# JCSaltFish/PBRPathTracer

Hardware: AMD Instinct MI355X
Metric: Msamples/s (pixels*spp/s) (higher is better)
Workload: dtype f32; 1 GPU; Cornell box (12 tris, no textures), 1280x720, 8 bounces, 256 spp; width=1280, height=720, max_depth=8, triangles=12, bvh_nodes=1, bvh_depth=1, parallelism=single GPU, exchange=none

## Files before the change

### include/ptk.h

```cpp
#ifndef PTK_H
#define PTK_H

#include <stddef.h>
#include <stdint.h>

#ifdef __cplusplus
extern "C" {
#endif

#define PTK_OK 0
#define PTK_ERR_BAD_ARG (-1)
#define PTK_ERR_HIP (-2)
#define PTK_ERR_RCCL (-3)
#define PTK_ERR_LIMIT (-4)

#define PTK_TILE 16
#ifndef PTK_MAX_BVH_DEPTH
#define PTK_MAX_BVH_DEPTH 32
#endif

typedef struct ptk_material {
    int32_t type;
    float diffuse[3];
    float specular[3];
// ... 418 lines not shown
int ptk_probe_unpack(ptk_ctx* ctx, int world, const float* host_packed , float* host_image);

int ptk_set_option(ptk_ctx* ctx, const char* name, double value);

int ptk_last_render_ms(ptk_ctx* ctx, float* ms, int* launches);
int ptk_last_kernel_ms(ptk_ctx* ctx, float* trace_ms, float* accumulate_ms);
int ptk_kernel_log(ptk_ctx* ctx, int capacity);
#define PTK_TRACE_NONE 0
#define PTK_TRACE_BVH 1
#define PTK_TRACE_FLAT 2
#define PTK_TRACE_FLAT_PLAIN 3
int ptk_trace_variant(ptk_ctx* ctx, int* variant);
int ptk_scene_is_plain(const ptk_scene_desc* scene);
int ptk_scene_is_lambert(const ptk_scene_desc* scene);
int ptk_trace_is_lambert(ptk_ctx* ctx, int* lambert);
int ptk_flat_zero_class(const float edges[6]);
int ptk_flat_zero_mask(int zero_class);
int ptk_flat_classes(ptk_ctx* ctx, int32_t out[16]);
int ptk_flat_rect_pair(const float rec_a[9], const float rec_b[9]);
int ptk_flat_rect_pairs(ptk_ctx* ctx, int32_t out[8], int32_t* num_pairs );
int ptk_kernel_log_read(ptk_ctx* ctx, float* trace_ms, int max_entries, int* num_entries);
int ptk_collect_stats(ptk_ctx* ctx, uint32_t first_sample, uint32_t spp_count, uint64_t seed, ptk_stats* out);
int ptk_bvh_info(ptk_ctx* ctx, int32_t* num_nodes, int32_t* depth , int32_t* num_leaf_tris);
int ptk_upload_timing(ptk_ctx* ctx, double* ms4, int* built_on_device );
int ptk_bvh_layout(ptk_ctx* ctx, int32_t* node_width, int32_t* node_bytes, int32_t* stack_need);

int ptk_download_bvh(ptk_ctx* ctx, float* nodes16, int32_t* leaf_order);

int ptk_probe_hits(ptk_ctx* ctx, int n, const float* ro, const float* rd, int32_t* tri, float* tuv);
int ptk_probe_primary_dirs(ptk_ctx* ctx, float* host_out );
// ... 8 lines not shown
```

### pbrpathtracer_amd/csrc/ptk_api.hip

```cpp
#include <hip/hip_runtime.h>
#include <hip/hip_gl_interop.h>
#include <dlfcn.h>

#include <algorithm>
#include <chrono>
#include <cmath>
#include <cstring>

#include "bvh_build.h"
#include "bvh_device.h"
#include "ptk_ctx.h"
#include "ptk_stage.h"
#include "ptk_device_fn.h"
#include "ptk_adaptive.h"
#include "ptk_refit.h"
#include "ptk_flat_mt.h"

using namespace ptk;

namespace {

inline float as_float(int32_t i) { float f; std::memcpy(&f, &i, 4); return f; }

void normalize3(const float* in, float* out)
// ... 180 lines not shown
struct AdaptiveRound
{
    AdaptiveParams a;
    ConvergeParams cp;
    bool init;
};

int run_passes(ptk_ctx* c, uint32_t first, uint32_t spp, uint64_t seed, bool stats, float* accum, uint8_t* rgb8,
               const uint32_t* exit_flag, bool timed, const AdaptiveRound* ad = nullptr)
{
    RenderParams p;
    fill_params(c, p, first, spp, seed);
    p.accum = accum; p.rgb8 = rgb8; p.exit_flag = exit_flag;
    if (const int rc = use_primary_cache(c, p); rc != PTK_OK) return rc;
    p.plain = (c->opt_plain_kernel && c->scene_plain && p.flat_count > 0 && p.primary_hit != nullptr) ? 1 : 0;
    if (p.plain && c->opt_flat_rect_pairs) p.plain = 2;
    p.lambert = (p.plain && c->opt_lambert_kernel && c->scene_lambert) ? 1 : 0;
    if (!c->pixel_rng_valid || c->pixel_rng_seed != seed)
    {
        launch_pixel_rng((uint32_t)seed, (uint32_t)(seed >> 32), c->width * c->height, c->d_pixel_rng, c->stream);
        HIPCHK(c, hipGetLastError());
        c->pixel_rng_seed = seed; c->pixel_rng_valid = true;
        c->inputs_dirty = true;
    }
    p.pixel_rng = c->d_pixel_rng;
    GlMapping glmap{ c };
    uint8_t* handoff = nullptr;
    if (rgb8 == c->d_rgb8)
    {
        handoff = c->out_host_dev ? c->out_host_dev : c->out_device;
        if (!handoff && c->gl_res)
// ... 133 lines not shown
        p.resolve_samples = (float)(first + done + n);
        const long long items = (long long)tiles * 4 * num_chunks;
        if (items > (1ll << 30)) return fail(c, PTK_ERR_LIMIT, "too many work items in one pass");
        p.num_items = (int)items;
        const int pi = c->last_passes < ptk_ctx::kMaxTimedPasses ? c->last_passes : -1;
        if (timed && pi >= 0) HIPCHK(c, hipEventRecord(c->ev[pi][0], tstream));
        const int kl = (!stats && (size_t)(2 * c->klog_n + 1) < c->klog_ev.size()) ? c->klog_n : -1;
        if (kl >= 0) HIPCHK(c, hipEventRecord(c->klog_ev[2 * kl], tstream));
        p.queues = overlap ? c->d_queues2[b] : c->d_queues;
        if (c->opt_contract == 1 && !stats) fma::launch_trace(p, tiles * 4, c->resident_waves, tstream, false);
        else if (c->opt_contract == 2 && !stats) fast::launch_trace(p, tiles * 4, c->resident_waves, tstream, false);
        else launch_trace(p, tiles * 4, c->resident_waves, tstream, stats);
        HIPCHK(c, hipGetLastError());
        c->last_trace_variant = p.flat_count <= 0 ? PTK_TRACE_BVH : ((p.plain && !stats) ? PTK_TRACE_FLAT_PLAIN : PTK_TRACE_FLAT);
        c->last_trace_lambert = p.flat_count > 0 && p.plain && p.lambert && !stats;
        if (timed && pi >= 0) HIPCHK(c, hipEventRecord(c->ev[pi][1], tstream));
        if (kl >= 0) { HIPCHK(c, hipEventRecord(c->klog_ev[2 * kl + 1], tstream)); c->klog_n = kl + 1; }
        if (overlap)
        {
            HIPCHK(c, hipEventRecord(c->ev_trace_done[b], tstream));
            HIPCHK(c, hipStreamWaitEvent(c->stream, c->ev_trace_done[b], 0));
        }
        if (ad) launch_accumulate_adaptive(p, ad->a, tiles, c->stream);
        else launch_accumulate(p, tiles, c->stream);
        HIPCHK(c, hipGetLastError());
        if (timed && pi >= 0) HIPCHK(c, hipEventRecord(c->ev[pi][2], c->stream));
        if (overlap)
        {
            HIPCHK(c, hipEventRecord(c->ev_acc_done[b], c->stream));
            c->acc_pending[b] = true;
// ... 543 lines not shown

int ptk_trace_variant(ptk_ctx* c, int* variant)
{
    if (!c || !variant) return PTK_ERR_BAD_ARG;
    *variant = c->last_trace_variant;
    return PTK_OK;
}

int ptk_trace_is_lambert(ptk_ctx* c, int* lambert)
{
    if (!c || !lambert) return PTK_ERR_BAD_ARG;
    *lambert = c->last_trace_lambert ? 1 : 0;
    return PTK_OK;
}

int ptk_set_camera(ptk_ctx* c, const float pos[3], const float dir[3], const float up[3],
                   float focal, float fovy_deg, float focal_dist, float aperture)
{
    if (!c || !pos || !dir || !up) return PTK_ERR_BAD_ARG;
    for (int a = 0; a < 3; a++)
        if (!(std::fabs(pos[a]) < 2.305843e18f)) return fail(c, PTK_ERR_LIMIT, "camera position is not finite or exceeds 2^61");
    for (int a = 0; a < 3; a++) c->cam_pos[a] = pos[a];
    normalize3(dir, c->cam_dir);
    normalize3(up, c->cam_up);
    c->focal = focal;
    if (c->focal <= 0.0f) c->focal = 0.1f;
    c->fovy = fovy_deg;
    if (c->fovy <= 0.0f) c->fovy = 0.1f;
    else if (c->fovy >= 180.0f) c->fovy = 179.5;
    c->focal_dist = focal_dist;
// ... 715 lines not shown
        return PTK_OK;
    }
    if (!std::strcmp(name, "flat_rect_pairs"))
    {
        const int use = value != 0.0 ? 1 : 0;
        if (use != c->opt_flat_rect_pairs && c->have_scene && c->d_flat_tris)
        {
            HIPCHK(c, hipSetDevice(c->device));
            launch_flat_classes(c->d_flat_tris, c->num_tris, c->opt_flat_zero_classes, use, c->stream);
            HIPCHK(c, hipGetLastError());
            c->inputs_dirty = true;
        }
        c->opt_flat_rect_pairs = use;
        return PTK_OK;
    }
    if (!std::strcmp(name, "device_build"))
    {
        c->opt_device_build = value != 0.0;
        return PTK_OK;
    }
    if (!std::strcmp(name, "primary_cache"))
    {
        c->opt_primary_cache = value != 0.0;
        return PTK_OK;
    }
    if (!std::strcmp(name, "pass_bytes"))
    {
        if (!(value >= 1 << 20 && value <= 32.0 * 1073741824.0)) return fail(c, PTK_ERR_BAD_ARG, "pass_bytes must be in [1 MiB, 32 GiB]");
        c->opt_pass_bytes = (size_t)value;
        return PTK_OK;
// ... 48 lines not shown
```

### pbrpathtracer_amd/csrc/ptk_ctx.h

```cpp
#pragma once
#include <hip/hip_runtime.h>

#include <atomic>
#include <mutex>
#include <string>
#include <vector>

#include "ptk_features.h"

typedef struct ncclComm* ncclComm_t;
namespace ptk { struct RaysBlock; }

struct ptk_ctx {
    int device = 0;
    hipStream_t stream = nullptr;
    bool own_stream = false;
    std::string error;
    std::mutex err_mu;

    float4* d_flat_tris = nullptr;
    float4 *d_nodes = nullptr, *d_tris = nullptr, *d_shade = nullptr, *d_mats = nullptr, *d_lights = nullptr;
    int4* d_texinfo = nullptr;
    uint32_t* d_texels = nullptr;
    int num_nodes = 0, num_tris = 0, num_lights = 0, bvh_depth = 0, bvh_stack = 0, num_leaf_tris = 0;
// ... 16 lines not shown
    float4* d_refit_side = nullptr;
    float* d_geo_stage = nullptr; size_t geo_stage_floats = 0;
    uint32_t* d_geo_red = nullptr;
    uint32_t* h_geo_red = nullptr;
    hipStream_t geo_stream = nullptr;
    hipEvent_t ev_geo_t[5] = { nullptr, nullptr, nullptr, nullptr, nullptr };
    bool geo_done_recorded = false, lights_stale = false;
    uint32_t geo_updates = 0;
    double sah_built = 0.0, sah_now = 0.0; bool sah_now_pending = false;
    float bvh_pad = 0.0f;
    bool scene_plain = false;
    int opt_plain_kernel = 1;
    bool scene_lambert = false;
    int opt_lambert_kernel = 1;
    int opt_flat_rect_pairs = 1;
    int opt_flat_zero_classes = 1;
    int last_trace_variant = PTK_TRACE_NONE;
    bool last_trace_lambert = false;

    float cam_pos[3] = { 0, 0, 0 }, cam_dir[3] = { 0, 0, 1 }, cam_up[3] = { 0, 1, 0 };
    float focal = 0.1f, fovy = 90.0f, focal_dist = 5.0f, aperture = 0.0f;
    float cam_right[3] = { 1, 0, 0 };
    bool primary_dirty = true;

    int width = 0, height = 0, max_depth = 3;
    float4* d_primary = nullptr;
    float4* d_primary_hit = nullptr;
    float4* d_primary_rd = nullptr;
    uint2* d_pixel_rng = nullptr;
    uint64_t pixel_rng_seed = 0; bool pixel_rng_valid = false;
    bool primary_hit_dirty = true, scene_has_opacity = false;
    int opt_primary_cache = 1;
// ... 253 lines not shown
```

### pbrpathtracer_amd/csrc/ptk_kernels.hip

```cpp

#include "ptk_device_fn.h"
#include "ptk_flat_mt.h"

namespace ptk {
#if PTK_CONTRACT >= 2
namespace fast {
#elif PTK_CONTRACT
namespace fma {
#endif

#define PTK_TRACE_BLOCK 64
#ifndef PTK_TRACE_WAVES
#define PTK_TRACE_WAVES 5
#endif
#ifndef PTK_TRACE_WAVES_PLAIN
#define PTK_TRACE_WAVES_PLAIN 5
#endif
#ifndef PTK_TRACE_WAVES_BVH
#define PTK_TRACE_WAVES_BVH 4
#endif

struct RayPair { f2 ox, oy, oz, dx, dy, dz; };

template <unsigned ZM>
// ... 225 lines not shown
    W.begin(camPos0, V(0.0f, 0.0f, 1.0f), 0, stack, 0.0f);
    W.occl_tri = -1;
    Walk WS;
    WS.begin(camPos0, V(0.0f, 0.0f, 1.0f), 0, stack, 0.0f);
    WS.occl_tri = -1;
    v3 L = V(0.0f, 0.0f, 0.0f), T = V(1.0f, 1.0f, 1.0f);
    v3 Tdi = V(0.0f, 0.0f, 0.0f), nextDir = V(0.0f, 0.0f, 1.0f);
    int depth = 0, iter = 0;
    bool inside = false;
    uint32_t ray = 0;
    int st = ST_NEED;

    float4* const samples_u = uniform_ptr(P.samples);
    const int num_nodes_u = __builtin_amdgcn_readfirstlane(P.num_nodes);
    const float scene_bound_u = __int_as_float(__builtin_amdgcn_readfirstlane(__float_as_int(P.scene_bound)));
#define PTK_FINISH_PATH()                                                                         \
    do {                                                                                          \
        samples_u[out_idx] = make_float4(L.x, L.y, L.z, 0.0f);                                    \
        st = ST_NEED;                                                                             \
    } while (0)

#define PTK_WALK_DONE()                                                                           \
    do {                                                                                          \
        if (STATS) { cnt.rays++; cnt.max_nodes = max(cnt.max_nodes, cnt.cur_nodes); cnt.cur_nodes = 0; }     \
        ray++;                                                                                    \
        const bool hit_ = W.best.tri != PTK_NOHIT;                                                \
        if (W.occl_tri >= 0)                                                                      \
        {                                                                                         \
                                \
            if (STATS) cnt.shadow++;                                                              \
            if (!(hit_ && W.best.tri != W.occl_tri)) L = add(L, Tdi);                             \
            W.occl_tri = -1;                                                                      \
            W.begin(W.ro, nextDir, num_nodes_u, stack, scene_bound_u);                                   \
        }                                                                                         \
        else if (!hit_ || (FLAT && !STATS && !((LAMBERT ? depth : iter) < P.max_depth))) PTK_FINISH_PATH();       \
        else st = ST_SHADE;                                                                       \
    } while (0)

    int debt_shade = 0, debt_gen = 0;
    for (;;)
    {
        bool deal = true;
        if (FLAT)
        {
            const int n_need = __popcll(__ballot(st == ST_NEED)), nt = __popcll(__ballot(st == ST_TRAV));
            const int ns = __popcll(__ballot(st == ST_SHADE)), ng = PLAIN ? 0 : __popcll(__ballot(st == ST_GEN));
            deal = nt == 0 || nt * 8 < (ns + n_need) * P.flat_shade_w || (!PLAIN && nt * 8 < (ng + n_need) * P.flat_gen_w);
        }
        if (!FLAT || deal)
        {
            unsigned long long m_need = __ballot(st == ST_NEED);
            while (m_need)
            {
// ... 24 lines not shown
        const unsigned long long m_gen = PLAIN ? 0ull : __ballot(st == ST_GEN);
        const int n_trav = __popcll(m_trav), n_shade = __popcll(m_shade), n_gen = __popcll(m_gen);
        const int n_live = n_trav + n_shade + n_gen;
        if (n_live == 0) break;

        bool run_shade = n_trav == 0 && n_shade >= n_gen && n_shade > 0;
        bool run_gen = n_trav == 0 && !run_shade;
        if (FLAT)
        {
            const int sc_trav = n_trav * 8, sc_shade = n_shade * P.flat_shade_w, sc_gen = n_gen * P.flat_gen_w;
            if (n_trav > 0 && sc_trav >= sc_shade && sc_trav >= sc_gen)
            {
                if (STATS && lane == 0) { cnt.walk_iters++; cnt.walk_lanes += (uint32_t)n_trav; }
                if (st == ST_TRAV)
                {
                    typedef float f4v __attribute__((ext_vector_type(4)));
                    typedef const __attribute__((address_space(4))) f4v* cf4;
                    const cf4 ct = (cf4)(uintptr_t)P.flat_tris;
                    const bool shadow = WS.occl_tri >= 0;
                    const uint32_t bounce_ray = shadow ? ray + 1u : ray;
                    RayPair R;
                    R.ox = f2{ W.ro.x, WS.ro.x }; R.oy = f2{ W.ro.y, WS.ro.y }; R.oz = f2{ W.ro.z, WS.ro.z };
                    R.dx = f2{ W.rd.x, WS.rd.x }; R.dy = f2{ W.rd.y, WS.rd.y }; R.dz = f2{ W.rd.z, WS.rd.z };
                    constexpr bool ZERO_CLASSES = PLAIN && !STATS && !PTK_CONTRACT;
                    typedef const __attribute__((address_space(4))) unsigned long long* cu64;
                    const unsigned long long classes = ZERO_CLASSES ? *(cu64)(uintptr_t)(P.flat_tris + FLAT_CLASSES_AT) : 0ull;
#ifdef PTK_RECT_UNIT
                    static_assert(ZERO_CLASSES, "the pair unit holds the exact PLAIN kernels only");
                    const unsigned long long pairs = *(cu64)(uintptr_t)(P.flat_tris + FLAT_PAIRS_AT);
                    const int n_pairs = (int)(pairs >> 32) & 15;
                    for (int j = 0; j < n_pairs; j++)
                    {
                        const f4v a0 = ct[j * 2 * TRI_F4], a1 = ct[j * 2 * TRI_F4 + 1], a2 = ct[j * 2 * TRI_F4 + 2];
                        f2 aA, uA, vA, tA, aB, uB, vB, tB;
#define PTK_RECT_KIND(c) tri_math_rect<c>(W, R, a0.x, a0.y, a0.z, a1.z, a1.w, a2.x, aA, uA, vA, tA, aB, uB, vB, tB); break;
                        switch ((unsigned)(pairs >> (j * 4)) & 15u)
                        {
                            case 1: PTK_RECT_KIND(1) case 2: PTK_RECT_KIND(2) case 3: PTK_RECT_KIND(3) case 4: PTK_RECT_KIND(4) case 5: PTK_RECT_KIND(5)
                            default: PTK_RECT_KIND(6)
                        }
#undef PTK_RECT_KIND
                        tri_accept_rect(W, WS, shadow, aA, tA, uA, vA, uB, vB, __float_as_int(a2.y));
                    }
                    for (int k = n_pairs * 2; k < P.flat_count; k++)
#else
                    for (int k = 0; k < P.flat_count; k++)
#endif
                    {
                        const f4v a0 = ct[k * TRI_F4], a1 = ct[k * TRI_F4 + 1], a2 = ct[k * TRI_F4 + 2];
                        const float4 t0 = make_float4(a0.x, a0.y, a0.z, a0.w), t1 = make_float4(a1.x, a1.y, a1.z, a1.w),
                                     t2 = make_float4(a2.x, a2.y, a2.z, a2.w);
#define PTK_ZERO_CLASS(c) case c: tri_math_pair<ZERO_CLASSES ? ptk_mt::flat_zero_mask(c) : 0u>(W, R, t0, t1, t2, ma, mu, mv, mt); break;
                        if (ZERO_CLASSES)
                        {
                            f2 ma, mu, mv, mt;
                            switch ((unsigned)(classes >> (k * 4)) & 15u)
                            {
                                PTK_ZERO_CLASS(1) PTK_ZERO_CLASS(2) PTK_ZERO_CLASS(3) PTK_ZERO_CLASS(4) PTK_ZERO_CLASS(5)
                                PTK_ZERO_CLASS(6) PTK_ZERO_CLASS(7) PTK_ZERO_CLASS(8) PTK_ZERO_CLASS(9) PTK_ZERO_CLASS(10)
                                PTK_ZERO_CLASS(11) PTK_ZERO_CLASS(12) PTK_ZERO_CLASS(13) PTK_ZERO_CLASS(14) PTK_ZERO_CLASS(15)
                                default: tri_math_pair<0u>(W, R, t0, t1, t2, ma, mu, mv, mt); break;
                            }
                            (void)tri_accept_pair<STATS, PLAIN>(P, W, WS, shadow, ma, mu, mv, mt, t2, rng, bounce_ray, ray, cnt);
                        }
                        else
                            (void)tri_test_pair<STATS, PLAIN>(P, W, WS, R, shadow, t0, t1, t2, rng, bounce_ray, ray, cnt);
#undef PTK_ZERO_CLASS
                    }
                    if (shadow)
                    {
                        if (STATS) { cnt.rays++; cnt.shadow++; }
                        if (!(WS.best.tri != PTK_NOHIT && WS.best.tri != WS.occl_tri)) L = add(L, Tdi);
                        WS.occl_tri = -1;
                        ray++;
                    }
                    W.node = NODE_EXIT;
                    PTK_WALK_DONE();
                }
                continue;
            }
            run_shade = n_shade > 0 && (sc_shade >= sc_gen || n_gen == 0);
            run_gen = !run_shade;
        }
        else if (n_trav > 0)
        {
            int ds = __builtin_amdgcn_readfirstlane(debt_shade), dg = __builtin_amdgcn_readfirstlane(debt_gen);
            unsigned long long m_tq = __ballot(W.tri_left > 0), m_nr = __ballot(W.node >= 0);
            bool want_shade = false, want_gen = false;
            const WalkParams WP = walk_params(P);
            NodeRec nrec;
            request_node(WP, W, nrec);
            do
// ... 16 lines not shown
                want_shade = (ns > 0) & (ds * 8 >= WP.shade_thr * (nl - ns));
                want_gen = (ng > 0) & (dg * 8 >= WP.gen_thr * (nl - ng));
                if (want_shade | want_gen | (nt == 0)) break;
            } while (true);
            if (want_shade) run_shade = true;
            else if (want_gen) run_gen = __ballot(st == ST_NEED) == 0ull;
            debt_shade = ds; debt_gen = dg;
            if (!run_shade && !run_gen) continue;
        }
        if (run_shade) debt_shade = 0; else debt_gen = 0;
        if (run_shade)
        {
            if (STATS) { const uint32_t nsx = (uint32_t)__popcll(__ballot(st == ST_SHADE)); if (lane == 0) { cnt.shade_execs++; cnt.shade_lanes += nsx; } }
            if (st == ST_SHADE)
            {
                if (depth < 0)
                {
                    const uint2 pr = P.pixel_rng[pix];
                    const float4 c = P.primary_hit[pix], r = P.primary_rd[pix];
                    rng.inc = pr.y;
                    rng.state = hash32(P.first_sample + sample_abs + pr.x);
                    rng.key = rng.state;
                    rng.state = rng.state * (747796405u * 747796405u) + rng.inc * (747796405u + 1u);
                    L = V(0.0f, 0.0f, 0.0f); T = V(1.0f, 1.0f, 1.0f);
                    depth = 0; iter = 0; inside = false; ray = 1;
                    W.occl_tri = -1;
                    if (STATS) cnt.started++;
                    W.ro = camPos0; W.rd = V(r.x, r.y, r.z);
                    W.best.tri = __float_as_int(c.x); W.best.t = c.y; W.best.u = c.z; W.best.v = c.w;
                    W.node = NODE_EXIT; W.top = stack; W.tri_left = 0;
                }
                const bool ended = shade_interaction<STATS, FLAT, PLAIN, LAMBERT>(P, W, WS, stack, rng, L, T, Tdi, nextDir, depth, iter, inside, ray, cnt);
                if (ended) PTK_FINISH_PATH();
                else st = ST_TRAV;
            }
        }
        else if (!PLAIN)
        {
            if (STATS) { const uint32_t ngx = (uint32_t)__popcll(__ballot(st == ST_GEN)); if (lane == 0) { cnt.gen_execs++; cnt.gen_lanes += ngx; } }
            if (st == ST_GEN)
            {
                const uint2 pr = P.pixel_rng[pix];
                const uint32_t pkey = pr.x;
                rng.inc = pr.y;
                rng.state = hash32(P.first_sample + sample_abs + pkey);
                rng.key = rng.state;
                L = V(0.0f, 0.0f, 0.0f); T = V(1.0f, 1.0f, 1.0f);
                depth = 0; iter = 0; inside = false; ray = 0;
                W.occl_tri = -1;
// ... 6 lines not shown
                if (P.aperture != 0.0f)
                {
                    float angle = (float)((double)r1 * 2. * PTK_PI_D);
                    float radius = sqrt_ieee(r2);
                    float sn, cs;
                    sincos_2pi(angle, sn, cs);
                    float offx = (cs * radius) * P.aperture, offy = (sn * radius) * P.aperture;
                    ro = add(camPos0, add(muls(camRight, offx), muls(camUp, offy)));
                }
                v3 rd = normalize(sub(focalPoint, ro));
                W.begin(ro, rd, P.num_nodes, stack, P.scene_bound);
                st = ST_TRAV;
            }
        }
    }
#undef PTK_WALK_DONE
#undef PTK_FINISH_PATH
    if (STATS)
    {
        atomicAdd(&P.stats[0], (unsigned long long)cnt.started);
        atomicAdd(&P.stats[1], (unsigned long long)cnt.rays);
        atomicAdd(&P.stats[2], (unsigned long long)cnt.shadow);
        atomicAdd(&P.stats[3], (unsigned long long)cnt.nodes);
        atomicAdd(&P.stats[4], (unsigned long long)cnt.tris);
        atomicAdd(&P.stats[5], (unsigned long long)cnt.shaded);
        atomicAdd(&P.stats[6], (unsigned long long)cnt.tex);
        atomicMax(&P.stats[15], (unsigned long long)cnt.max_nodes);
        if (lane == 0)
        {
            atomicAdd(&P.stats[7], (unsigned long long)cnt.walk_iters);
            atomicAdd(&P.stats[8], (unsigned long long)cnt.walk_lanes);
            atomicAdd(&P.stats[9], (unsigned long long)cnt.shade_execs);
            atomicAdd(&P.stats[10], (unsigned long long)cnt.shade_lanes);
            atomicAdd(&P.stats[11], (unsigned long long)cnt.gen_execs);
            atomicAdd(&P.stats[12], (unsigned long long)cnt.gen_lanes);
            atomicAdd(&P.stats[13], (unsigned long long)cnt.tri_execs);
            atomicAdd(&P.stats[14], (unsigned long long)cnt.tri_lanes);
        }
    }
}

#if !PTK_CONTRACT
void launch_trace_plain(bool lambert, int blocks, hipStream_t stream, const RenderParams* dp);
void launch_trace_rect(bool lambert, int blocks, hipStream_t stream, const RenderParams* dp);
#endif
#ifdef PTK_PLAIN_UNIT
#if PTK_CONTRACT
#error "the PLAIN unit belongs to the exact build: the contracted builds keep their PLAIN kernels in ptk_kernels.hip"
#endif
#ifdef PTK_RECT_UNIT
void launch_trace_rect(bool lambert, int blocks, hipStream_t stream, const RenderParams* dp)
#else
void launch_trace_plain(bool lambert, int blocks, hipStream_t stream, const RenderParams* dp)
#endif
{
    if (lambert) hipLaunchKernelGGL((trace_kernel<false, true, true, true>), dim3(blocks), dim3(PTK_TRACE_BLOCK), 0, stream, dp);
    else hipLaunchKernelGGL((trace_kernel<false, true, true>), dim3(blocks), dim3(PTK_TRACE_BLOCK), 0, stream, dp);
}
#else

__global__ __launch_bounds__(PTK_BLOCK) void probe_math_kernel(int op, const float* __restrict__ in, float* __restrict__ out, int n)
{
    const int i = blockIdx.x * PTK_BLOCK + threadIdx.x;
    if (i >= n) return;
    const float x = in[i];
// ... 48 lines not shown
    QueueGeometry geo = {};
    geo.w[QG_NUM_CHUNKS] = p.num_chunks; geo.w[QG_WORLD] = p.world; geo.w[QG_RANK] = p.rank;
    geo.w[QG_TILES_X] = p.tiles_x; geo.w[QG_CHUNK] = p.chunk; geo.w[QG_SPP] = (int)p.spp;
    if (!(p.flat_count > 0) && PTK_TRACE_WAVES_BVH != 4) resident_waves = resident_waves / 16 * 4 * PTK_TRACE_WAVES_BVH;
    if (p.flat_count > 0 && PTK_TRACE_WAVES != 4) resident_waves = resident_waves / 16 * 4 * ((p.plain && !stats) ? PTK_TRACE_WAVES_PLAIN : PTK_TRACE_WAVES);
    if (p.persistent < 0) p.persistent = padded > 4 * resident_waves ? 1 : 0;
    const int generations = p.persistent ? std::max(1, std::min(p.generations, padded / resident_waves)) : 1;
    const int blocks = p.persistent ? resident_waves * generations : padded;
    geo.w[QG_QUOTA] = generations > 1 ? blocks : 0;
    hipLaunchKernelGGL(queue_init_kernel, dim3(1), dim3(64), 0, stream, p.queues, geo, p.live_count, p);
    const RenderParams* dp = queue_block_params(p.queues);
    const bool flat = p.flat_count > 0;
#if !PTK_CONTRACT
    if (stats && flat) hipLaunchKernelGGL((trace_kernel<true, true, false>), dim3(blocks), dim3(PTK_TRACE_BLOCK), 0, stream, dp);
    else if (stats) hipLaunchKernelGGL((trace_kernel<true, false, false>), dim3(blocks), dim3(PTK_TRACE_BLOCK), 0, stream, dp);
    else if (flat && p.plain == 2) launch_trace_rect(p.lambert != 0, blocks, stream, dp);
    else if (flat && p.plain) launch_trace_plain(p.lambert != 0, blocks, stream, dp);
    else
#else
    if (flat && p.plain && p.lambert) hipLaunchKernelGGL((trace_kernel<false, true, true, true>), dim3(blocks), dim3(PTK_TRACE_BLOCK), 0, stream, dp);
    else if (flat && p.plain) hipLaunchKernelGGL((trace_kernel<false, true, true>), dim3(blocks), dim3(PTK_TRACE_BLOCK), 0, stream, dp);
    else
#endif
    if (flat) hipLaunchKernelGGL((trace_kernel<false, true, false>), dim3(blocks), dim3(PTK_TRACE_BLOCK), 0, stream, dp);
    else hipLaunchKernelGGL((trace_kernel<false, false, false>), dim3(blocks), dim3(PTK_TRACE_BLOCK), 0, stream, dp);
}

#endif

#if PTK_CONTRACT
// ... 4 lines not shown
```

### pbrpathtracer_amd/ptk.py

```python
from __future__ import annotations

import ctypes as C
import threading
import os
from typing import Optional

import numpy as np

_HERE = os.path.dirname(os.path.abspath(__file__))
LIB_PATH = os.path.join(_HERE, "libptk.so")
if os.environ.get("PTK_DEV_TOOLS") == "1" and os.environ.get("PTK_LIB_PATH", "").startswith(os.path.join(_HERE, "libptk_")):
    LIB_PATH = os.environ["PTK_LIB_PATH"]

PTK_OK = 0
PTK_TILE = 16
PTK_MAX_BVH_DEPTH = 32

MATERIAL_DTYPE = np.dtype([
    ("type", np.int32), ("diffuse", np.float32, 3), ("specular", np.float32, 3),
    ("emissive", np.float32, 3), ("emissive_intensity", np.float32), ("roughness", np.float32),
    ("reflectiveness", np.float32), ("translucency", np.float32), ("ior", np.float32),
    ("tex", np.int32, 6)], align=False)
TEXTURE_DTYPE = np.dtype([("width", np.int32), ("height", np.int32), ("offset", np.int64)])
assert MATERIAL_DTYPE.itemsize == 84 and TEXTURE_DTYPE.itemsize == 16
# ... 104 lines not shown


_lib = None

SYMBOLS = [
    "ptk_create", "ptk_destroy", "ptk_upload_scene", "ptk_update_materials", "ptk_set_camera", "ptk_set_frame", "ptk_set_tile",
    "ptk_reset", "ptk_render", "ptk_resolve_rgb8", "ptk_read_accum", "ptk_write_accum", "ptk_samples",
    "ptk_request_exit", "ptk_synchronize", "ptk_last_error", "ptk_accum_device_ptr", "ptk_rgb8_device_ptr",
    "ptk_bind_accum", "ptk_set_stream", "ptk_gather_accum", "ptk_set_option", "ptk_last_render_ms",
    "ptk_last_kernel_ms", "ptk_collect_stats",
    "ptk_bvh_info", "ptk_bvh_layout", "ptk_upload_timing", "ptk_download_bvh", "ptk_probe_hits", "ptk_probe_primary_dirs", "ptk_probe_math", "ptk_probe_direct", "ptk_host_alloc", "ptk_host_free",
    "ptk_packed_floats", "ptk_packed_layout", "ptk_comm_unique_id", "ptk_comm_init", "ptk_comm_destroy",
    "ptk_gather_wait", "ptk_read_gathered", "ptk_gathered_device_ptr", "ptk_probe_pack", "ptk_probe_unpack",
    "ptk_bind_out_image", "ptk_bind_out_device", "ptk_bind_gl_buffer", "ptk_comm_info", "ptk_kernel_log", "ptk_kernel_log_read",
    "ptk_debug_stall_exchange", "ptk_render_adaptive", "ptk_read_sample_counts", "ptk_read_moments",
    "ptk_trace_variant", "ptk_scene_is_plain", "ptk_scene_is_lambert", "ptk_trace_is_lambert",
    "ptk_flat_zero_class", "ptk_flat_zero_mask", "ptk_flat_classes", "ptk_flat_rect_pair", "ptk_flat_rect_pairs",
    "ptk_feature_info", "ptk_render_features", "ptk_read_feature", "ptk_feature_device_ptr", "ptk_pick",
    "ptk_update_geometry", "ptk_update_geometry_device", "ptk_geometry_info", "ptk_geometry_timing",
    "ptk_trace_rays", "ptk_trace_rays_device", "ptk_last_rays_ms",
    "ptk_intersect_rays", "ptk_intersect_rays_device", "ptk_occluded_rays", "ptk_occluded_rays_device", "ptk_last_hits_ms",
    "ptk_closest_points", "ptk_closest_points_device", "ptk_last_closest_ms", "ptk_closest_stats",
    "ptk_crossings_rays", "ptk_crossings_rays_device", "ptk_contains_points", "ptk_contains_points_device",
    "ptk_inside_default_dirs", "ptk_signed_distance", "ptk_signed_distance_device", "ptk_last_crossings_ms",
    "ptk_multihit_rays", "ptk_multihit_rays_device", "ptk_last_multihit_ms",
    "ptk_denoise_planes", "ptk_denoise_planes_device", "ptk_denoise_frame", "ptk_read_denoised", "ptk_denoised_device_ptr",
    "ptk_resolve_denoised_rgb8", "ptk_last_denoise_ms",
    "ptk_get_view", "ptk_reproject_planes", "ptk_reproject_planes_device", "ptk_temporal_frame", "ptk_read_temporal",
    "ptk_temporal_device_ptr", "ptk_last_temporal_ms",
    "ptk_geometry_snapshot", "ptk_render_motion", "ptk_read_motion", "ptk_motion_device_ptr", "ptk_reproject_planes_moving",
    "ptk_reproject_planes_moving_device", "ptk_temporal_frame_moving", "ptk_last_motion_ms",
# ... 171 lines not shown
        L.ptk_display_srgb_table.argtypes = [vp]
        L.ptk_display_check_params.argtypes = [C.POINTER(DisplayParams)]
        L.ptk_last_display_ms.argtypes = [vp, fp, fp, fp]
        L.ptk_render_guides.argtypes = [vp, i32, i32, u32, u64, u32]
        L.ptk_read_guide.argtypes = [vp, i32, vp]
        L.ptk_guide_device_ptr.argtypes = [vp, i32, C.POINTER(vp), C.POINTER(C.c_size_t)]
        L.ptk_guide_view.argtypes = [vp, C.POINTER(View)]
        for fn in (L.ptk_upsample_planes, L.ptk_upsample_planes_device):
            fn.argtypes = [vp, i32, i32] + [vp] * 5 + [i32, i32] + [vp] * 4 + [C.POINTER(UpsampleParams), vp, vp]
        L.ptk_upsample_frame.argtypes = [vp, i32, C.POINTER(UpsampleParams)]
        L.ptk_read_upsampled.argtypes = [vp, vp, vp]
        L.ptk_upsampled_device_ptr.argtypes = [vp, C.POINTER(vp), C.POINTER(vp), C.POINTER(C.c_int), C.POINTER(C.c_int)]
        L.ptk_last_upsample_ms.argtypes = [vp, fp, fp]
        L.ptk_scene_is_lambert.argtypes = [C.POINTER(SceneDesc)]
        L.ptk_trace_is_lambert.argtypes = [vp, C.POINTER(C.c_int)]
        L.ptk_flat_zero_class.argtypes = [C.POINTER(C.c_float)]
        L.ptk_flat_zero_mask.argtypes = [C.c_int]
        L.ptk_flat_classes.argtypes = [vp, C.POINTER(i32)]
        L.ptk_flat_rect_pair.argtypes = [C.POINTER(C.c_float), C.POINTER(C.c_float)]
        L.ptk_flat_rect_pairs.argtypes = [vp, C.POINTER(i32), C.POINTER(i32)]
    except AttributeError:
        if LIB_PATH.endswith("libptk.so"):
            raise
    L.ptk_feature_info.argtypes = [i32, C.POINTER(i32), C.POINTER(i32)]
    L.ptk_render_features.argtypes = [vp, u32, u64, u32]
    L.ptk_read_feature.argtypes = [vp, i32, vp]
    L.ptk_feature_device_ptr.argtypes = [vp, i32, C.POINTER(vp), C.POINTER(C.c_size_t)]
    L.ptk_pick.argtypes = [vp, i32, i32, u64, C.POINTER(C.c_int32), C.POINTER(C.c_int32), C.POINTER(C.c_float)]
    L.ptk_update_geometry.argtypes = [vp, C.c_int32, C.c_int32, vp, vp, vp]
    L.ptk_update_geometry_device.argtypes = [vp, C.c_int32, C.c_int32, vp, vp, vp]
    L.ptk_geometry_info.argtypes = [vp, C.POINTER(C.c_uint32), C.POINTER(C.c_int), C.POINTER(C.c_double), C.POINTER(C.c_double)]
    L.ptk_geometry_timing.argtypes = [vp, C.POINTER(C.c_float)]
    L.ptk_bvh_info.argtypes = [vp, C.POINTER(C.c_int32), C.POINTER(C.c_int32), C.POINTER(C.c_int32)]
    L.ptk_bvh_layout.argtypes = [vp, C.POINTER(C.c_int32), C.POINTER(C.c_int32), C.POINTER(C.c_int32)]
    L.ptk_download_bvh.argtypes = [vp, vp, vp]
    L.ptk_upload_timing.argtypes = [vp, C.POINTER(C.c_double), C.POINTER(C.c_int)]
    L.ptk_probe_hits.argtypes = [vp, i32, vp, vp, vp, vp]
    L.ptk_probe_math.argtypes = [vp, i32, i32, vp, vp]
    L.ptk_probe_direct.argtypes = [vp, i32, vp, vp, vp, vp, vp]
    L.ptk_probe_primary_dirs.argtypes = [vp, vp]
    _lib = L
    return L


TRACE_NONE, TRACE_BVH, TRACE_FLAT, TRACE_FLAT_PLAIN = 0, 1, 2, 3
RAYS_ACCUMULATE, RAYS_LENS_DRAWS = 1, 2
BAKE_ACCUMULATE, BAKE_BACK = 1, 2
PROBES_ACCUMULATE = 1
DENOISE_VARIANCE = 1
INSIDE_WINDING, INSIDE_PARITY = 0, 1
MULTIHIT_MAX = 16
INSIDE_MODES = {"winding": INSIDE_WINDING, "parity": INSIDE_PARITY}


def inside_default_dirs() -> np.ndarray:
    out = np.zeros((3, 3), np.float32)
    if load().ptk_inside_default_dirs(out.ctypes.data) != PTK_OK:
        raise PtkError("ptk_inside_default_dirs failed")
    return out

# ... 1263 lines not shown
        cap = max(1, getattr(self, "_klog_cap", 0))
        buf = (C.c_float * cap)(); n = C.c_int(0)
        self._chk(self.L.ptk_kernel_log_read(self.h, buf, cap, C.byref(n)), "ptk_kernel_log_read")
        return [float(buf[i]) for i in range(n.value)]

    def trace_variant(self) -> int:
        v = C.c_int(0)
        self._chk(self.L.ptk_trace_variant(self.h, C.byref(v)), "ptk_trace_variant")
        return v.value

    def trace_is_lambert(self) -> bool:
        v = C.c_int(0)
        self._chk(self.L.ptk_trace_is_lambert(self.h, C.byref(v)), "ptk_trace_is_lambert")
        return bool(v.value)

    def flat_classes(self) -> list:
        out = (C.c_int32 * 16)()
        self._chk(self.L.ptk_flat_classes(self.h, out), "ptk_flat_classes")
        return [int(v) for v in out if v >= 0]

    def flat_rect_pairs(self) -> list:
        out = (C.c_int32 * 8)()
        m = C.c_int32(0)
        self._chk(self.L.ptk_flat_rect_pairs(self.h, out, C.byref(m)), "ptk_flat_rect_pairs")
        return [int(out[k]) for k in range(m.value)]

    def set_option(self, name: str, value: float):
        self._chk(self.L.ptk_set_option(self.h, name.encode(), float(value)), "ptk_set_option")

    def collect_stats(self, first_sample: int, spp: int, seed: int) -> dict:
# ... 147 lines not shown
```

Measured before the change: 72640 Msamples/s.

## Add cycle trace unit with simplified shade/trace loop and uniform scalar params

Adds a third PLAIN kernel variant (cycle unit), enabled by default. It replaces the general state-machine scheduler with a tight loop: refill idle lanes with new sample units via ballot/mbcnt, then shade, then run a flat-triangle pass. Work-item fields and kernel parameters are read with readfirstlane so they stay in scalar registers. The aim is to cut scheduler overhead and divergence in the persistent trace kernel. The cost is an extra kernel build and possibly different refill behaviour when the queue runs dry.

New measurement: 79330 Msamples/s (median of 6 runs). 1.09x the previous value.

```diff
diff --git a/include/ptk.h b/include/ptk.h
--- a/include/ptk.h
+++ b/include/ptk.h
@@ -456,6 +456,11 @@
 int ptk_scene_is_plain(const ptk_scene_desc* scene);
 int ptk_scene_is_lambert(const ptk_scene_desc* scene);
 int ptk_trace_is_lambert(ptk_ctx* ctx, int* lambert);
+#define PTK_UNIT_NONE 0
+#define PTK_UNIT_PLAIN 1
+#define PTK_UNIT_RECT 2
+#define PTK_UNIT_CYCLE 3
+int ptk_trace_unit(ptk_ctx* ctx, int* unit);
 int ptk_flat_zero_class(const float edges[6]);
 int ptk_flat_zero_mask(int zero_class);
 int ptk_flat_classes(ptk_ctx* ctx, int32_t out[16]);
diff --git a/pbrpathtracer_amd/csrc/ptk_api.hip b/pbrpathtracer_amd/csrc/ptk_api.hip
--- a/pbrpathtracer_amd/csrc/ptk_api.hip
+++ b/pbrpathtracer_amd/csrc/ptk_api.hip
@@ -218,7 +218,7 @@
     p.accum = accum; p.rgb8 = rgb8; p.exit_flag = exit_flag;
     if (const int rc = use_primary_cache(c, p); rc != PTK_OK) return rc;
     p.plain = (c->opt_plain_kernel && c->scene_plain && p.flat_count > 0 && p.primary_hit != nullptr) ? 1 : 0;
-    if (p.plain && c->opt_flat_rect_pairs) p.plain = 2;
+    if (p.plain && c->opt_flat_rect_pairs) p.plain = c->opt_flat_cycle ? 3 : 2;
     p.lambert = (p.plain && c->opt_lambert_kernel && c->scene_lambert) ? 1 : 0;
     if (!c->pixel_rng_valid || c->pixel_rng_seed != seed)
     {
@@ -382,6 +382,7 @@
         HIPCHK(c, hipGetLastError());
         c->last_trace_variant = p.flat_count <= 0 ? PTK_TRACE_BVH : ((p.plain && !stats) ? PTK_TRACE_FLAT_PLAIN : PTK_TRACE_FLAT);
         c->last_trace_lambert = p.flat_count > 0 && p.plain && p.lambert && !stats;
+        c->last_trace_unit = (p.flat_count > 0 && p.plain && !stats && c->opt_contract == 0) ? (p.plain == 3 ? PTK_UNIT_CYCLE : p.plain == 2 ? PTK_UNIT_RECT : PTK_UNIT_PLAIN) : PTK_UNIT_NONE;
         if (timed && pi >= 0) HIPCHK(c, hipEventRecord(c->ev[pi][1], tstream));
         if (kl >= 0) { HIPCHK(c, hipEventRecord(c->klog_ev[2 * kl + 1], tstream)); c->klog_n = kl + 1; }
         if (overlap)
@@ -955,6 +956,13 @@
     return PTK_OK;
 }
 
+int ptk_trace_unit(ptk_ctx* c, int* unit)
+{
+    if (!c || !unit) return PTK_ERR_BAD_ARG;
+    *unit = c->last_trace_unit;
+    return PTK_OK;
+}
+
 int ptk_set_camera(ptk_ctx* c, const float pos[3], const float dir[3], const float up[3],
                    float focal, float fovy_deg, float focal_dist, float aperture)
 {
@@ -1700,6 +1708,11 @@
         c->opt_flat_rect_pairs = use;
         return PTK_OK;
     }
+    if (!std::strcmp(name, "flat_cycle"))
+    {
+        c->opt_flat_cycle = value != 0.0 ? 1 : 0;
+        return PTK_OK;
+    }
     if (!std::strcmp(name, "device_build"))
     {
         c->opt_device_build = value != 0.0;
diff --git a/pbrpathtracer_amd/csrc/ptk_ctx.h b/pbrpathtracer_amd/csrc/ptk_ctx.h
--- a/pbrpathtracer_amd/csrc/ptk_ctx.h
+++ b/pbrpathtracer_amd/csrc/ptk_ctx.h
@@ -54,8 +54,10 @@
     bool scene_lambert = false;
     int opt_lambert_kernel = 1;
     int opt_flat_rect_pairs = 1;
+    int opt_flat_cycle = 1;
     int opt_flat_zero_classes = 1;
     int last_trace_variant = PTK_TRACE_NONE;
+    int last_trace_unit = PTK_UNIT_NONE;
     bool last_trace_lambert = false;
 
     float cam_pos[3] = { 0, 0, 0 }, cam_dir[3] = { 0, 0, 1 }, cam_up[3] = { 0, 1, 0 };
diff --git a/pbrpathtracer_amd/csrc/ptk_kernels.hip b/pbrpathtracer_amd/csrc/ptk_kernels.hip
--- a/pbrpathtracer_amd/csrc/ptk_kernels.hip
+++ b/pbrpathtracer_amd/csrc/ptk_kernels.hip
@@ -263,6 +263,12 @@
     float4* const samples_u = uniform_ptr(P.samples);
     const int num_nodes_u = __builtin_amdgcn_readfirstlane(P.num_nodes);
     const float scene_bound_u = __int_as_float(__builtin_amdgcn_readfirstlane(__float_as_int(P.scene_bound)));
+#ifdef PTK_CYCLE_UNIT
+    const int max_depth_u = __builtin_amdgcn_readfirstlane(P.max_depth);
+#define PTK_U_MAX_DEPTH max_depth_u
+#else
+#define PTK_U_MAX_DEPTH P.max_depth
+#endif
 #define PTK_FINISH_PATH()                                                                         \
     do {                                                                                          \
         samples_u[out_idx] = make_float4(L.x, L.y, L.z, 0.0f);                                    \
@@ -282,10 +288,13 @@
             W.occl_tri = -1;                                                                      \
             W.begin(W.ro, nextDir, num_nodes_u, stack, scene_bound_u);                                   \
         }                                                                                         \
-        else if (!hit_ || (FLAT && !STATS && !((LAMBERT ? depth : iter) < P.max_depth))) PTK_FINISH_PATH();       \
+        else if (!hit_ || (FLAT && !STATS && !((LAMBERT ? depth : iter) < PTK_U_MAX_DEPTH))) PTK_FINISH_PATH();       \
         else st = ST_SHADE;                                                                       \
     } while (0)
 
+#ifdef PTK_CYCLE_UNIT
+#include "ptk_trace_cycle.h"
+#else
     int debt_shade = 0, debt_gen = 0;
     for (;;)
     {
@@ -340,68 +349,7 @@
                 if (STATS && lane == 0) { cnt.walk_iters++; cnt.walk_lanes += (uint32_t)n_trav; }
                 if (st == ST_TRAV)
                 {
-                    typedef float f4v __attribute__((ext_vector_type(4)));
-                    typedef const __attribute__((address_space(4))) f4v* cf4;
-                    const cf4 ct = (cf4)(uintptr_t)P.flat_tris;
-                    const bool shadow = WS.occl_tri >= 0;
-                    const uint32_t bounce_ray = shadow ? ray + 1u : ray;
-                    RayPair R;
-                    R.ox = f2{ W.ro.x, WS.ro.x }; R.oy = f2{ W.ro.y, WS.ro.y }; R.oz = f2{ W.ro.z, WS.ro.z };
-                    R.dx = f2{ W.rd.x, WS.rd.x }; R.dy = f2{ W.rd.y, WS.rd.y }; R.dz = f2{ W.rd.z, WS.rd.z };
-                    constexpr bool ZERO_CLASSES = PLAIN && !STATS && !PTK_CONTRACT;
-                    typedef const __attribute__((address_space(4))) unsigned long long* cu64;
-                    const unsigned long long classes = ZERO_CLASSES ? *(cu64)(uintptr_t)(P.flat_tris + FLAT_CLASSES_AT) : 0ull;
-#ifdef PTK_RECT_UNIT
-                    static_assert(ZERO_CLASSES, "the pair unit holds the exact PLAIN kernels only");
-                    const unsigned long long pairs = *(cu64)(uintptr_t)(P.flat_tris + FLAT_PAIRS_AT);
-                    const int n_pairs = (int)(pairs >> 32) & 15;
-                    for (int j = 0; j < n_pairs; j++)
-                    {
-                        const f4v a0 = ct[j * 2 * TRI_F4], a1 = ct[j * 2 * TRI_F4 + 1], a2 = ct[j * 2 * TRI_F4 + 2];
-                        f2 aA, uA, vA, tA, aB, uB, vB, tB;
-#define PTK_RECT_KIND(c) tri_math_rect<c>(W, R, a0.x, a0.y, a0.z, a1.z, a1.w, a2.x, aA, uA, vA, tA, aB, uB, vB, tB); break;
-                        switch ((unsigned)(pairs >> (j * 4)) & 15u)
-                        {
-                            case 1: PTK_RECT_KIND(1) case 2: PTK_RECT_KIND(2) case 3: PTK_RECT_KIND(3) case 4: PTK_RECT_KIND(4) case 5: PTK_RECT_KIND(5)
-                            default: PTK_RECT_KIND(6)
-                        }
-#undef PTK_RECT_KIND
-                        tri_accept_rect(W, WS, shadow, aA, tA, uA, vA, uB, vB, __float_as_int(a2.y));
-                    }
-                    for (int k = n_pairs * 2; k < P.flat_count; k++)
-#else
-                    for (int k = 0; k < P.flat_count; k++)
-#endif
-                    {
-                        const f4v a0 = ct[k * TRI_F4], a1 = ct[k * TRI_F4 + 1], a2 = ct[k * TRI_F4 + 2];
-                        const float4 t0 = make_float4(a0.x, a0.y, a0.z, a0.w), t1 = make_float4(a1.x, a1.y, a1.z, a1.w),
-                                     t2 = make_float4(a2.x, a2.y, a2.z, a2.w);
-#define PTK_ZERO_CLASS(c) case c: tri_math_pair<ZERO_CLASSES ? ptk_mt::flat_zero_mask(c) : 0u>(W, R, t0, t1, t2, ma, mu, mv, mt); break;
-                        if (ZERO_CLASSES)
-                        {
-                            f2 ma, mu, mv, mt;
-                            switch ((unsigned)(classes >> (k * 4)) & 15u)
-                            {
-                                PTK_ZERO_CLASS(1) PTK_ZERO_CLASS(2) PTK_ZERO_CLASS(3) PTK_ZERO_CLASS(4) PTK_ZERO_CLASS(5)
-                                PTK_ZERO_CLASS(6) PTK_ZERO_CLASS(7) PTK_ZERO_CLASS(8) PTK_ZERO_CLASS(9) PTK_ZERO_CLASS(10)
-                                PTK_ZERO_CLASS(11) PTK_ZERO_CLASS(12) PTK_ZERO_CLASS(13) PTK_ZERO_CLASS(14) PTK_ZERO_CLASS(15)
-                                default: tri_math_pair<0u>(W, R, t0, t1, t2, ma, mu, mv, mt); break;
-                            }
-                            (void)tri_accept_pair<STATS, PLAIN>(P, W, WS, shadow, ma, mu, mv, mt, t2, rng, bounce_ray, ray, cnt);
-                        }
-                        else
-                            (void)tri_test_pair<STATS, PLAIN>(P, W, WS, R, shadow, t0, t1, t2, rng, bounce_ray, ray, cnt);
-#undef PTK_ZERO_CLASS
-                    }
-                    if (shadow)
-                    {
-                        if (STATS) { cnt.rays++; cnt.shadow++; }
-                        if (!(WS.best.tri != PTK_NOHIT && WS.best.tri != WS.occl_tri)) L = add(L, Tdi);
-                        WS.occl_tri = -1;
-                        ray++;
-                    }
-                    W.node = NODE_EXIT;
-                    PTK_WALK_DONE();
+#include "ptk_trace_pass.h"
                 }
                 continue;
             }
@@ -448,25 +396,7 @@
             if (STATS) { const uint32_t nsx = (uint32_t)__popcll(__ballot(st == ST_SHADE)); if (lane == 0) { cnt.shade_execs++; cnt.shade_lanes += nsx; } }
             if (st == ST_SHADE)
             {
-                if (depth < 0)
-                {
-                    const uint2 pr = P.pixel_rng[pix];
-                    const float4 c = P.primary_hit[pix], r = P.primary_rd[pix];
-                    rng.inc = pr.y;
-                    rng.state = hash32(P.first_sample + sample_abs + pr.x);
-                    rng.key = rng.state;
-                    rng.state = rng.state * (747796405u * 747796405u) + rng.inc * (747796405u + 1u);
-                    L = V(0.0f, 0.0f, 0.0f); T = V(1.0f, 1.0f, 1.0f);
-                    depth = 0; iter = 0; inside = false; ray = 1;
-                    W.occl_tri = -1;
-                    if (STATS) cnt.started++;
-                    W.ro = camPos0; W.rd = V(r.x, r.y, r.z);
-                    W.best.tri = __float_as_int(c.x); W.best.t = c.y; W.best.u = c.z; W.best.v = c.w;
-                    W.node = NODE_EXIT; W.top = stack; W.tri_left = 0;
-                }
-                const bool ended = shade_interaction<STATS, FLAT, PLAIN, LAMBERT>(P, W, WS, stack, rng, L, T, Tdi, nextDir, depth, iter, inside, ray, cnt);
-                if (ended) PTK_FINISH_PATH();
-                else st = ST_TRAV;
+#include "ptk_trace_shade.h"
             }
         }
         else if (!PLAIN)
@@ -503,8 +433,10 @@
             }
         }
     }
+#endif
 #undef PTK_WALK_DONE
 #undef PTK_FINISH_PATH
+#undef PTK_U_MAX_DEPTH
     if (STATS)
     {
         atomicAdd(&P.stats[0], (unsigned long long)cnt.started);
@@ -532,12 +464,15 @@
 #if !PTK_CONTRACT
 void launch_trace_plain(bool lambert, int blocks, hipStream_t stream, const RenderParams* dp);
 void launch_trace_rect(bool lambert, int blocks, hipStream_t stream, const RenderParams* dp);
+void launch_trace_cycle(bool lambert, int blocks, hipStream_t stream, const RenderParams* dp);
 #endif
 #ifdef PTK_PLAIN_UNIT
 #if PTK_CONTRACT
 #error "the PLAIN unit belongs to the exact build: the contracted builds keep their PLAIN kernels in ptk_kernels.hip"
 #endif
-#ifdef PTK_RECT_UNIT
+#if defined(PTK_CYCLE_UNIT)
+void launch_trace_cycle(bool lambert, int blocks, hipStream_t stream, const RenderParams* dp)
+#elif defined(PTK_RECT_UNIT)
 void launch_trace_rect(bool lambert, int blocks, hipStream_t stream, const RenderParams* dp)
 #else
 void launch_trace_plain(bool lambert, int blocks, hipStream_t stream, const RenderParams* dp)
@@ -616,6 +551,7 @@
 #if !PTK_CONTRACT
     if (stats && flat) hipLaunchKernelGGL((trace_kernel<true, true, false>), dim3(blocks), dim3(PTK_TRACE_BLOCK), 0, stream, dp);
     else if (stats) hipLaunchKernelGGL((trace_kernel<true, false, false>), dim3(blocks), dim3(PTK_TRACE_BLOCK), 0, stream, dp);
+    else if (flat && p.plain == 3) launch_trace_cycle(p.lambert != 0, blocks, stream, dp);
     else if (flat && p.plain == 2) launch_trace_rect(p.lambert != 0, blocks, stream, dp);
     else if (flat && p.plain) launch_trace_plain(p.lambert != 0, blocks, stream, dp);
     else
diff --git a/pbrpathtracer_amd/csrc/ptk_kernels_cycle.hip b/pbrpathtracer_amd/csrc/ptk_kernels_cycle.hip
--- /dev/null
+++ b/pbrpathtracer_amd/csrc/ptk_kernels_cycle.hip
@@ -0,0 +1,6 @@
+#include "ptk_unit_map.h"
+#define PTK_PLAIN_UNIT 1
+#define PTK_RECT_UNIT 1
+#define PTK_CYCLE_UNIT 1
+#define trace_kernel trace_kernel_cycle
+#include "ptk_kernels.hip"
diff --git a/pbrpathtracer_amd/csrc/ptk_trace_cycle.h b/pbrpathtracer_amd/csrc/ptk_trace_cycle.h
--- /dev/null
+++ b/pbrpathtracer_amd/csrc/ptk_trace_cycle.h
@@ -0,0 +1,75 @@
+    static_assert(PLAIN && !STATS && FLAT, "the cycle unit holds the exact PLAIN kernels only");
+    (void)camRight; (void)camUp;
+    {
+        const uint32_t width_u = (uint32_t)__builtin_amdgcn_readfirstlane(P.width);
+        const float4* const flat_tris_u = uniform_ptr(P.flat_tris);
+        const int flat_count_u = __builtin_amdgcn_readfirstlane(P.flat_count);
+#define PTK_U_FLAT_TRIS flat_tris_u
+#define PTK_U_FLAT_COUNT flat_count_u
+        uint32_t it_nlive = 1u, it_magic = 0u, it_pixbase = 0u, it_sbegin = 0u, it_outbase = 0u;
+        uint32_t dry = 0u;
+        auto take_unit = [&](uint32_t u)
+        {
+            const UnitPlace up = unit_place(u, it_nlive, it_magic, lds_pixel_of_rank, it_outbase);
+            pix = unit_pixel(up.q, it_pixbase, width_u);
+            sample_abs = it_sbegin + up.s;
+            out_idx = up.slot;
+            st = ST_SHADE;
+            depth = -1;
+        };
+        for (;;)
+        {
+            unsigned long long m_need = __ballot(st == ST_NEED);
+            if (m_need)
+            {
+                uint32_t wanted = (uint32_t)__popcll(m_need);
+                if (wanted > total_units - next_unit)
+                {
+                    for (;;)
+                    {
+                        if (next_unit >= total_units)
+                        {
+                            next_unit = 0u;
+                            total_units = dry ? 0u : (uint32_t)__builtin_amdgcn_readfirstlane((int)acquire_item());
+                            if (total_units == 0u)
+                            {
+                                dry = 1u;
+                                if (__builtin_amdgcn_inverse_ballot_w64(m_need)) st = ST_DONE;
+                                wanted = 0u;
+                                break;
+                            }
+                            it_nlive = (uint32_t)__builtin_amdgcn_readfirstlane((int)lds_item[IT_NLIVE]);
+                            it_magic = (uint32_t)__builtin_amdgcn_readfirstlane((int)lds_item[IT_NLIVE_MAGIC]);
+                            it_pixbase = (uint32_t)__builtin_amdgcn_readfirstlane((int)lds_item[IT_Y0]) * width_u + (uint32_t)__builtin_amdgcn_readfirstlane((int)lds_item[IT_X0]);
+                            it_sbegin = (uint32_t)__builtin_amdgcn_readfirstlane((int)lds_item[IT_SBEGIN]);
+                            it_outbase = (uint32_t)__builtin_amdgcn_readfirstlane((int)lds_item[IT_OUTBASE]);
+                        }
+                        const uint32_t avail = total_units - next_unit;
+                        if (wanted <= avail) break;
+                        const uint32_t rank = __builtin_amdgcn_mbcnt_hi((uint32_t)(m_need >> 32), __builtin_amdgcn_mbcnt_lo((uint32_t)m_need, 0u));
+                        if (__builtin_amdgcn_inverse_ballot_w64(m_need) && rank < avail) take_unit(next_unit + rank);
+                        next_unit = total_units;
+                        m_need = __ballot(st == ST_NEED);
+                        wanted = (uint32_t)__popcll(m_need);
+                    }
+                }
+                if (wanted)
+                {
+                    const uint32_t rank = __builtin_amdgcn_mbcnt_hi((uint32_t)(m_need >> 32), __builtin_amdgcn_mbcnt_lo((uint32_t)m_need, 0u));
+                    if (__builtin_amdgcn_inverse_ballot_w64(m_need)) take_unit(next_unit + rank);
+                    next_unit += wanted;
+                }
+            }
+            if (__ballot(st == ST_SHADE) == 0ull) break;
+            if (st == ST_SHADE)
+            {
+#include "ptk_trace_shade.h"
+            }
+            if (st == ST_TRAV)
+            {
+#include "ptk_trace_pass.h"
+            }
+        }
+#undef PTK_U_FLAT_TRIS
+#undef PTK_U_FLAT_COUNT
+    }
diff --git a/pbrpathtracer_amd/csrc/ptk_trace_pass.h b/pbrpathtracer_amd/csrc/ptk_trace_pass.h
--- /dev/null
+++ b/pbrpathtracer_amd/csrc/ptk_trace_pass.h
@@ -0,0 +1,68 @@
+#ifndef PTK_U_FLAT_TRIS
+#define PTK_U_FLAT_TRIS P.flat_tris
+#endif
+#ifndef PTK_U_FLAT_COUNT
+#define PTK_U_FLAT_COUNT P.flat_count
+#endif
+                    typedef float f4v __attribute__((ext_vector_type(4)));
+                    typedef const __attribute__((address_space(4))) f4v* cf4;
+                    const cf4 ct = (cf4)(uintptr_t)PTK_U_FLAT_TRIS;
+                    const bool shadow = WS.occl_tri >= 0;
+                    const uint32_t bounce_ray = shadow ? ray + 1u : ray;
+                    RayPair R;
+                    R.ox = f2{ W.ro.x, WS.ro.x }; R.oy = f2{ W.ro.y, WS.ro.y }; R.oz = f2{ W.ro.z, WS.ro.z };
+                    R.dx = f2{ W.rd.x, WS.rd.x }; R.dy = f2{ W.rd.y, WS.rd.y }; R.dz = f2{ W.rd.z, WS.rd.z };
+                    constexpr bool ZERO_CLASSES = PLAIN && !STATS && !PTK_CONTRACT;
+                    typedef const __attribute__((address_space(4))) unsigned long long* cu64;
+                    const unsigned long long classes = ZERO_CLASSES ? *(cu64)(uintptr_t)(PTK_U_FLAT_TRIS + FLAT_CLASSES_AT) : 0ull;
+#ifdef PTK_RECT_UNIT
+                    static_assert(ZERO_CLASSES, "the pair unit holds the exact PLAIN kernels only");
+                    const unsigned long long pairs = *(cu64)(uintptr_t)(PTK_U_FLAT_TRIS + FLAT_PAIRS_AT);
+                    const int n_pairs = (int)(pairs >> 32) & 15;
+                    for (int j = 0; j < n_pairs; j++)
+                    {
+                        const f4v a0 = ct[j * 2 * TRI_F4], a1 = ct[j * 2 * TRI_F4 + 1], a2 = ct[j * 2 * TRI_F4 + 2];
+                        f2 aA, uA, vA, tA, aB, uB, vB, tB;
+#define PTK_RECT_KIND(c) tri_math_rect<c>(W, R, a0.x, a0.y, a0.z, a1.z, a1.w, a2.x, aA, uA, vA, tA, aB, uB, vB, tB); break;
+                        switch ((unsigned)(pairs >> (j * 4)) & 15u)
+                        {
+                            case 1: PTK_RECT_KIND(1) case 2: PTK_RECT_KIND(2) case 3: PTK_RECT_KIND(3) case 4: PTK_RECT_KIND(4) case 5: PTK_RECT_KIND(5)
+                            default: PTK_RECT_KIND(6)
+                        }
+#undef PTK_RECT_KIND
+                        tri_accept_rect(W, WS, shadow, aA, tA, uA, vA, uB, vB, __float_as_int(a2.y));
+                    }
+                    for (int k = n_pairs * 2; k < PTK_U_FLAT_COUNT; k++)
+#else
+                    for (int k = 0; k < PTK_U_FLAT_COUNT; k++)
+#endif
+                    {
+                        const f4v a0 = ct[k * TRI_F4], a1 = ct[k * TRI_F4 + 1], a2 = ct[k * TRI_F4 + 2];
+                        const float4 t0 = make_float4(a0.x, a0.y, a0.z, a0.w), t1 = make_float4(a1.x, a1.y, a1.z, a1.w),
+                                     t2 = make_float4(a2.x, a2.y, a2.z, a2.w);
+#define PTK_ZERO_CLASS(c) case c: tri_math_pair<ZERO_CLASSES ? ptk_mt::flat_zero_mask(c) : 0u>(W, R, t0, t1, t2, ma, mu, mv, mt); break;
+                        if (ZERO_CLASSES)
+                        {
+                            f2 ma, mu, mv, mt;
+                            switch ((unsigned)(classes >> (k * 4)) & 15u)
+                            {
+                                PTK_ZERO_CLASS(1) PTK_ZERO_CLASS(2) PTK_ZERO_CLASS(3) PTK_ZERO_CLASS(4) PTK_ZERO_CLASS(5)
+                                PTK_ZERO_CLASS(6) PTK_ZERO_CLASS(7) PTK_ZERO_CLASS(8) PTK_ZERO_CLASS(9) PTK_ZERO_CLASS(10)
+                                PTK_ZERO_CLASS(11) PTK_ZERO_CLASS(12) PTK_ZERO_CLASS(13) PTK_ZERO_CLASS(14) PTK_ZERO_CLASS(15)
+                                default: tri_math_pair<0u>(W, R, t0, t1, t2, ma, mu, mv, mt); break;
+                            }
+                            (void)tri_accept_pair<STATS, PLAIN>(P, W, WS, shadow, ma, mu, mv, mt, t2, rng, bounce_ray, ray, cnt);
+                        }
+                        else
+                            (void)tri_test_pair<STATS, PLAIN>(P, W, WS, R, shadow, t0, t1, t2, rng, bounce_ray, ray, cnt);
+#undef PTK_ZERO_CLASS
+                    }
+                    if (shadow)
+                    {
+                        if (STATS) { cnt.rays++; cnt.shadow++; }
+                        if (!(WS.best.tri != PTK_NOHIT && WS.best.tri != WS.occl_tri)) L = add(L, Tdi);
+                        WS.occl_tri = -1;
+                        ray++;
+                    }
+                    W.node = NODE_EXIT;
+                    PTK_WALK_DONE();
diff --git a/pbrpathtracer_amd/csrc/ptk_trace_shade.h b/pbrpathtracer_amd/csrc/ptk_trace_shade.h
--- /dev/null
+++ b/pbrpathtracer_amd/csrc/ptk_trace_shade.h
@@ -0,0 +1,19 @@
+                if (depth < 0)
+                {
+                    const uint2 pr = P.pixel_rng[pix];
+                    const float4 c = P.primary_hit[pix], r = P.primary_rd[pix];
+                    rng.inc = pr.y;
+                    rng.state = hash32(P.first_sample + sample_abs + pr.x);
+                    rng.key = rng.state;
+                    rng.state = rng.state * (747796405u * 747796405u) + rng.inc * (747796405u + 1u);
+                    L = V(0.0f, 0.0f, 0.0f); T = V(1.0f, 1.0f, 1.0f);
+                    depth = 0; iter = 0; inside = false; ray = 1;
+                    W.occl_tri = -1;
+                    if (STATS) cnt.started++;
+                    W.ro = camPos0; W.rd = V(r.x, r.y, r.z);
+                    W.best.tri = __float_as_int(c.x); W.best.t = c.y; W.best.u = c.z; W.best.v = c.w;
+                    W.node = NODE_EXIT; W.top = stack; W.tri_left = 0;
+                }
+                const bool ended = shade_interaction<STATS, FLAT, PLAIN, LAMBERT>(P, W, WS, stack, rng, L, T, Tdi, nextDir, depth, iter, inside, ray, cnt);
+                if (ended) PTK_FINISH_PATH();
+                else st = ST_TRAV;
diff --git a/pbrpathtracer_amd/csrc/ptk_unit_map.h b/pbrpathtracer_amd/csrc/ptk_unit_map.h
--- /dev/null
+++ b/pbrpathtracer_amd/csrc/ptk_unit_map.h
@@ -0,0 +1,28 @@
+#pragma once
+#include <stdint.h>
+
+#if defined(__HIPCC__) || defined(__CUDACC__)
+#define PTK_UNIT_MAP_FN __host__ __device__ inline __attribute__((always_inline))
+#else
+#define PTK_UNIT_MAP_FN inline
+#endif
+
+namespace ptk {
+
+struct UnitPlace { uint32_t q, s, slot; };
+
+PTK_UNIT_MAP_FN uint32_t unit_magic(uint32_t n_live) { return (uint32_t)((0x100000000ull + n_live - 1u) / n_live); }
+
+template <class Table>
+PTK_UNIT_MAP_FN UnitPlace unit_place(uint32_t u, uint32_t n_live, uint32_t magic, const Table& pixel_of_rank, uint32_t out_base)
+{
+    UnitPlace p;
+    p.s = n_live == 1u ? u : (uint32_t)(((uint64_t)u * magic) >> 32);
+    p.q = (uint32_t)pixel_of_rank[u - p.s * n_live];
+    p.slot = out_base + p.s * 64u + p.q;
+    return p;
+}
+
+PTK_UNIT_MAP_FN uint32_t unit_pixel(uint32_t q, uint32_t base, uint32_t width) { return base + (q >> 3) * width + (q & 7u); }
+
+}
diff --git a/pbrpathtracer_amd/ptk.py b/pbrpathtracer_amd/ptk.py
--- a/pbrpathtracer_amd/ptk.py
+++ b/pbrpathtracer_amd/ptk.py
@@ -142,7 +142,7 @@
     "ptk_gather_wait", "ptk_read_gathered", "ptk_gathered_device_ptr", "ptk_probe_pack", "ptk_probe_unpack",
     "ptk_bind_out_image", "ptk_bind_out_device", "ptk_bind_gl_buffer", "ptk_comm_info", "ptk_kernel_log", "ptk_kernel_log_read",
     "ptk_debug_stall_exchange", "ptk_render_adaptive", "ptk_read_sample_counts", "ptk_read_moments",
-    "ptk_trace_variant", "ptk_scene_is_plain", "ptk_scene_is_lambert", "ptk_trace_is_lambert",
+    "ptk_trace_variant", "ptk_scene_is_plain", "ptk_scene_is_lambert", "ptk_trace_is_lambert", "ptk_trace_unit",
     "ptk_flat_zero_class", "ptk_flat_zero_mask", "ptk_flat_classes", "ptk_flat_rect_pair", "ptk_flat_rect_pairs",
     "ptk_feature_info", "ptk_render_features", "ptk_read_feature", "ptk_feature_device_ptr", "ptk_pick",
     "ptk_update_geometry", "ptk_update_geometry_device", "ptk_geometry_info", "ptk_geometry_timing",
@@ -344,6 +344,7 @@
         L.ptk_last_upsample_ms.argtypes = [vp, fp, fp]
         L.ptk_scene_is_lambert.argtypes = [C.POINTER(SceneDesc)]
         L.ptk_trace_is_lambert.argtypes = [vp, C.POINTER(C.c_int)]
+        L.ptk_trace_unit.argtypes = [vp, C.POINTER(C.c_int)]
         L.ptk_flat_zero_class.argtypes = [C.POINTER(C.c_float)]
         L.ptk_flat_zero_mask.argtypes = [C.c_int]
         L.ptk_flat_classes.argtypes = [vp, C.POINTER(i32)]
@@ -374,6 +375,7 @@
 
 
 TRACE_NONE, TRACE_BVH, TRACE_FLAT, TRACE_FLAT_PLAIN = 0, 1, 2, 3
+UNIT_NONE, UNIT_PLAIN, UNIT_RECT, UNIT_CYCLE = 0, 1, 2, 3
 RAYS_ACCUMULATE, RAYS_LENS_DRAWS = 1, 2
 BAKE_ACCUMULATE, BAKE_BACK = 1, 2
 PROBES_ACCUMULATE = 1
@@ -1667,6 +1669,11 @@
         self._chk(self.L.ptk_trace_is_lambert(self.h, C.byref(v)), "ptk_trace_is_lambert")
         return bool(v.value)
 
+    def trace_unit(self) -> int:
+        v = C.c_int(0)
+        self._chk(self.L.ptk_trace_unit(self.h, C.byref(v)), "ptk_trace_unit")
+        return v.value
+
     def flat_classes(self) -> list:
         out = (C.c_int32 * 16)()
         self._chk(self.L.ptk_flat_classes(self.h, out), "ptk_flat_classes")
```
